# abstractguy/xagents

Hardware: AMD Instinct MI355X
Metric: env-steps/sec/GPU (PPO 16-env) + update ms; 1/2/4/8 MI355X (higher is better)
Workload: dtype f32; 1 GPU; PPO CartPole-v1, 16 envs/GPU, MLP[64,64], n_steps=128, 4 epochs x 4 minibatches, synthetic obs replay (the metric's 16-env configuration); the replay records ignore the actions, so the rollout runs its policy forwards as one batched launch (the `dynamics` object times the sequential step loop of an action-dependent env); n_envs_per_gpu=16, n_steps=128, batch_per_gpu=2048, minibatch_per_gpu=512, ppo_epochs=4, parallelism=dp1, graph=True, train_steps_per_graph_replay=8, update=persistent, allreduce=none

## Files before the change

xagents_amd/csrc/ppo_update_impl.hpp:

```cpp
#pragma once
#include <math.h>
#include <stdlib.h>

#include "../../include/xagents_hip.h"
#include "ppo_tile.hpp"
#include "xa_adam.hpp"
#include "xa_common.hpp"

__device__ void xa_forms_not_unrolled()
    __attribute__((error("ppo_update_kernel: the step loop's forms were not unrolled")));

namespace {

using namespace xa_ac;
using namespace xa_pt;

typedef __attribute__((address_space(1))) unsigned gu32;
typedef __attribute__((address_space(1))) unsigned long long gu64;

constexpr int kMaxSteps = 128;
constexpr int kCtlBytes = 256;
constexpr uint64_t kSpinTicks = 1000000000;
constexpr int kXcds = 8;
enum { kCntStats = 0, kAbort = 1 };
// ... 111 lines not shown
  return __longlong_as_double((long long)((u & ~1ull) | (unsigned long long)(tag & 1u)));
}
XA_DEV void st_d2_tagged(__amdgpu_buffer_rsrc_t r, uint32_t off, double a, double b, unsigned tag) {
  st_wt_d2(r, off, d_tagged(a, tag), d_tagged(b, tag));
}
XA_DEV bool d2_ok(const double2& v, unsigned tag) {
  return ((((unsigned)__double_as_longlong(v.x)) ^ tag) & 1u) == 0u &&
         ((((unsigned)__double_as_longlong(v.y)) ^ tag) & 1u) == 0u;
}

#ifndef XA_POLL_SLEEP
#define XA_POLL_SLEEP 1
#endif
template <int N>
XA_DEV bool poll_gran(__amdgpu_buffer_rsrc_t r, const uint32_t (&off)[N], int n, unsigned tag,
                      f32x4v (&v)[N], unsigned* ctl, unsigned epoch, int* status) {
  uint64_t t0 = 0;
  for (unsigned it = 0;; ++it) {
    const bool slow = (it & 15u) == 15u;
#pragma unroll
    for (int u = 0; u < N; ++u)
      if (u < n) v[u] = __builtin_amdgcn_raw_buffer_load_b128(r, off[u], 0, kAuxSc1);
    const unsigned ab = slow ? __hip_atomic_load((gu32*)(ctl + kAbort), __ATOMIC_RELAXED,
                                                 __HIP_MEMORY_SCOPE_AGENT)
                             : 0u;
    bool ok = true;
#pragma unroll
    for (int u = 0; u < N; ++u)
      if (u < n) ok = ok && gran_ok(v[u], tag);
    if (ok) return true;
    if (!slow) {
#ifndef XA_POLL_NOSLEEP
      __builtin_amdgcn_s_sleep(XA_POLL_SLEEP);
#endif
      continue;
    }
    if (ab == epoch) return false;
    {
      const uint64_t now = wall_clock64();
      if (t0 == 0) t0 = now;
      else if (now - t0 > kSpinTicks) {
        __hip_atomic_store((gu32*)(ctl + kAbort), epoch, __ATOMIC_RELAXED, __HIP_MEMORY_SCOPE_AGENT);
        if (status) __hip_atomic_store((gu32*)status, 1u, __ATOMIC_RELAXED, __HIP_MEMORY_SCOPE_AGENT);
        return false;
      }
    }
  }
}

template <int N>
XA_DEV bool poll_row(__amdgpu_buffer_rsrc_t r, const uint32_t (&off)[N], int n, unsigned tag,
                     RowG (&v)[N], unsigned* ctl, unsigned epoch, int* status) {
  uint64_t t0 = 0;
  for (unsigned it = 0;; ++it) {
    const bool slow = (it & 15u) == 15u;
#pragma unroll
    for (int u = 0; u < N; ++u)
      if (u < n) v[u] = ld_row(r, off[u]);
    const unsigned ab = slow ? __hip_atomic_load((gu32*)(ctl + kAbort), __ATOMIC_RELAXED,
                                                 __HIP_MEMORY_SCOPE_AGENT)
                             : 0u;
    bool ok = true;
#pragma unroll
    for (int u = 0; u < N; ++u)
      if (u < n) ok = ok && row_ok(v[u], tag);
    if (ok) return true;
    if (!slow) {
#ifndef XA_POLL_NOSLEEP
      __builtin_amdgcn_s_sleep(XA_POLL_SLEEP);
#endif
      continue;
    }
    if (ab == epoch) return false;
    {
      const uint64_t now = wall_clock64();
      if (t0 == 0) t0 = now;
      else if (now - t0 > kSpinTicks) {
        __hip_atomic_store((gu32*)(ctl + kAbort), epoch, __ATOMIC_RELAXED, __HIP_MEMORY_SCOPE_AGENT);
        if (status) __hip_atomic_store((gu32*)status, 1u, __ATOMIC_RELAXED, __HIP_MEMORY_SCOPE_AGENT);
        return false;
      }
    }
  }
}

template <int N>
XA_DEV bool poll_d2(__amdgpu_buffer_rsrc_t r, const uint32_t (&off)[N], uint32_t valid,
                    unsigned tag, double2 (&v)[N], unsigned* ctl, unsigned epoch, int* status) {
  uint64_t t0 = 0;
  for (unsigned it = 0;; ++it) {
    const bool slow = (it & 15u) == 15u;
#pragma unroll
    for (int u = 0; u < N; ++u)
      if ((valid >> u) & 1u) v[u] = ld_wt_d2(r, off[u]);
    const unsigned ab = slow ? __hip_atomic_load((gu32*)(ctl + kAbort), __ATOMIC_RELAXED,
                                                 __HIP_MEMORY_SCOPE_AGENT)
                             : 0u;
    bool ok = true;
#pragma unroll
    for (int u = 0; u < N; ++u)
      if ((valid >> u) & 1u) ok = ok && d2_ok(v[u], tag);
    if (ok) return true;
    if (!slow) {
#ifndef XA_POLL_NOSLEEP
      __builtin_amdgcn_s_sleep(XA_POLL_SLEEP);
#endif
      continue;
    }
    if (ab == epoch) return false;
    {
      const uint64_t now = wall_clock64();
      if (t0 == 0) t0 = now;
      else if (now - t0 > kSpinTicks) {
        __hip_atomic_store((gu32*)(ctl + kAbort), epoch, __ATOMIC_RELAXED, __HIP_MEMORY_SCOPE_AGENT);
        if (status) __hip_atomic_store((gu32*)status, 1u, __ATOMIC_RELAXED, __HIP_MEMORY_SCOPE_AGENT);
        return false;
      }
    }
  }
}

XA_DEV int xcc_id() {
  unsigned x;
  asm volatile("s_getreg_b32 %0, hwreg(HW_REG_XCC_ID)" : "=s"(x));
  return (int)(x & (kXcds - 1));
}

#ifdef XA_TRACE
constexpr int kTraceSteps = 32, kTracePts = 16;
__device__ unsigned xa_ppo_trace[256 * kTraceSteps * kTracePts];
#define XA_TRACE_PT(blk, k, i)                                                        \
  do {                                                                                \
    if (threadIdx.x == 0 && (k) < kTraceSteps) {                                      \
      unsigned long long t_;                                                          \
      asm volatile("s_memrealtime %0\n\ts_waitcnt lgkmcnt(0)" : "=s"(t_)::"memory");  \
      U.trace[(k) * kTracePts + (i)] = (unsigned)t_;                                  \
    }                                                                                 \
  } while (0)
#define XA_TRACE_CLK(blk, i)                                                          \
  do {                                                                                \
    if (threadIdx.x == 0) {                                                           \
      unsigned long long t_, c_;                                                      \
      asm volatile("s_memrealtime %0\n\ts_memtime %1\n\ts_waitcnt lgkmcnt(0)"        \
                   : "=s"(t_), "=s"(c_)::"memory");                                   \
      U.trace[(kTraceSteps - 1) * kTracePts + 8 + 2 * (i)] = (unsigned)t_;            \
      U.trace[(kTraceSteps - 1) * kTracePts + 9 + 2 * (i)] = (unsigned)c_;            \
    }                                                                                 \
  } while (0)
#define XA_TRACE_FLUSH(blk)                                                           \
  do {                                                                                \
    __syncthreads();                                                                  \
    for (int i_ = threadIdx.x; i_ < kTraceSteps * kTracePts; i_ += 256)              \
      xa_ppo_trace[(size_t)(blk) * kTraceSteps * kTracePts + i_] = U.trace[i_];      \
  } while (0)
#else
#define XA_TRACE_PT(blk, k, i) \
  do {                         \
  } while (0)
#define XA_TRACE_CLK(blk, i) \
  do {                       \
  } while (0)
#define XA_TRACE_FLUSH(blk) \
  do {                      \
  } while (0)
#endif

// ... 75 lines not shown
                    uint32_t (&w)[N], unsigned* ctl, unsigned epoch, int* status) {
  uint64_t t0 = 0;
  for (unsigned it = 0;; ++it) {
    const bool slow = (it & 15u) == 15u;
    bool ok = true;
#pragma unroll
    for (int u = 0; u < N; ++u)
      if (u < n) {
        const unsigned long long v = dp_ld(base, off[u]);
        w[u] = (uint32_t)v;
        ok = ok && (unsigned)(v >> 32) == tag;
      }
    const unsigned ab = slow ? __hip_atomic_load((gu32*)(ctl + kAbort), __ATOMIC_RELAXED,
                                                 __HIP_MEMORY_SCOPE_AGENT)
                             : 0u;
    if (ok) return true;
    if (slow) {
      if (ab == epoch) return false;
      const uint64_t now = wall_clock64();
      if (t0 == 0) t0 = now;
      else if (now - t0 > kSpinTicks) {
        __hip_atomic_store((gu32*)(ctl + kAbort), epoch, __ATOMIC_RELAXED, __HIP_MEMORY_SCOPE_AGENT);
        if (status) __hip_atomic_store((gu32*)status, 1u, __ATOMIC_RELAXED, __HIP_MEMORY_SCOPE_AGENT);
        return false;
      }
    }
    __builtin_amdgcn_s_sleep(XA_POLL_SLEEP);
  }
}

struct ShufKeys {
  uint32_t k[4];
  uint32_t half_bits;
};

XA_DEV ShufKeys shuf_keys(const XaShuffle& sh, uint64_t ctr, int epoch, int batch) {
  ShufKeys s;
  const xa_u4 r = xa_philox((uint32_t)epoch, 0x5u, (uint32_t)ctr, (uint32_t)(ctr >> 32),
                            (uint32_t)sh.seed, (uint32_t)(sh.seed >> 32));
  s.k[0] = r.x;
  s.k[1] = r.y;
  s.k[2] = r.z;
  s.k[3] = r.w;
  const uint32_t bits = batch <= 1 ? 1u : 32u - __clz((uint32_t)(batch - 1));
  s.half_bits = (bits + 1u) / 2u;
  if (s.half_bits == 0) s.half_bits = 1;
  return s;
}

XA_DEV int shuf_index(const XaShuffle& sh, const ShufKeys& keys, int epoch, int batch, int g) {
  if (sh.perm) return sh.perm[(size_t)epoch * batch + g];
  return (int)xa_permute((uint32_t)g, (uint32_t)batch, keys.half_bits, keys.k[0], keys.k[1],
                         keys.k[2], keys.k[3]);
}

constexpr int kPreBytes = 16384;
template <int OBS>
constexpr int pre_max() { return kPreBytes / ((OBS + 4) * 4); }

constexpr int kBF = 11;
template <int OBS, int A, int TS>
struct UpdLds {
  PtLds<OBS, A, TS> t;
  alignas(16) float row[(offs(OBS, A).P + 3) & ~3];
  alignas(16) float pre[pre_max<OBS>() * (OBS + 4)];
  alignas(16) float stage[TS * (OBS + 4)];
  alignas(16) float scr_own[TS == 32 ? 4 : 2 * 256 * kBF];
  XA_DEV float* scr() {
    static_assert(TS != 32 || (H + 2 * TS) * LDW + H * PtLds<OBS, A, TS>::LDT >= 2 * 256 * kBF,
                  "gather scratch");
    return TS == 32 ? t.sH1 : scr_own;
  }
  static constexpr int NS = 16 + Dims<OBS, A>::RPT, NQ4 = (NS + 3) / 4;
  float4 mv4[2][NQ4][256];
  float alpha[kMaxSteps];
  float stat[kMaxSteps][4];
  double red[256 * 4];
  double wsum[4];
  int flag;
  int xn[kXcds];
  int wx[4][kXcds];
  int xmem[256];
  int xrank;
#ifdef XA_TRACE
  unsigned trace[kTraceSteps * kTracePts];
#endif
};

constexpr int kLocForceWt = 2;

struct UniF {
  float b1, b2, eps, clip, omb1, omb2;
};
struct NoUniF {
  static constexpr float b1 = 0.0f, b2 = 0.0f, eps = 0.0f, clip = 0.0f, omb1 = 0.0f, omb2 = 0.0f;
};
XA_DEV float uni_vreg(float x) {
  float r;
  asm volatile("v_mov_b32 %0, %1" : "=v"(r) : "s"(x));
  return r;
}
XA_DEV float uni_clip_scale(float clip, float gn) {
  asm volatile("" : "+v"(clip));
  return clip > 0.0f ? clip * fminf(frcp(gn), frcp(clip)) : 1.0f;
}
template <bool ON>
XA_DEV int uni_tid(int tid) {
  if constexpr (ON) asm volatile("" : "+v"(tid));
  return tid;
}
template <bool ON>
XA_DEV auto uni_ptid(int tid) {
  if constexpr (ON) {
    asm volatile("" : "+v"(tid));
    return tid;
  } else {
    return PtOwnTid{};
  }
}


template <int BF>
struct FixShape {
  static constexpr int B = BF == 3 ? 2048 : 32768, MB = BF == 3 ? 512 : 8192, K = 16, NMB = 4;
  static constexpr int G = BF == 3 ? 32 : 256;
};
template <int OBS, int A, int TS, bool DP, bool PRE, int BF = 0>
__global__ __launch_bounds__(256) void ppo_update_kernel(XaPpoUpdateArgs p, Ws ws, int K_,
                                                          int n_mb_, int loc_) {
  constexpr bool FIX = BF == 3 || BF == 4;
  typedef FixShape<BF> FS;
  const int K = FIX ? FS::K : K_, n_mb = FIX ? FS::NMB : n_mb_;
  const int loc = (BF == 2 || BF == 4) ? 0 : loc_;
  if (loc && ((int)blockIdx.x & (kXcds - 1)) != 0) return;
  constexpr int RPT = Dims<OBS, A>::RPT;
  __shared__ __attribute__((aligned(16))) UpdLds<OBS, A, TS> U;
  PtLds<OBS, A, TS>& L = U.t;
  const Offs o = offs(OBS, A);
  const int P = o.P;
  const int tid = threadIdx.x, lane = tid & 63, w = tid >> 6;
  XA_STAMP_DECL
#ifdef XA_TRACE
  unsigned long long t_entry_;
  asm volatile("s_memrealtime %0\n\ts_waitcnt lgkmcnt(0)" : "=s"(t_entry_)::"memory");
#endif

  const unsigned gen =
      __hip_atomic_load((gu32*)ws.persist, __ATOMIC_RELAXED, __HIP_MEMORY_SCOPE_AGENT);
  const unsigned epoch = gen + 1u;
  const int xcc = xcc_id();
  const int G = FIX ? FS::G : loc ? p.n_blocks : (int)gridDim.x;
  const int b = loc ? (int)blockIdx.x / kXcds : (int)blockIdx.x;
#ifdef XA_TRACE
  if (tid == 0) U.trace[(kTraceSteps - 1) * kTracePts + 5] = (unsigned)t_entry_;
#endif
  constexpr int kSW = 2;
  const unsigned* const st_src = static_cast<const unsigned*>(p.stats_src);
  unsigned* const st_dst =
      p.stats_words > 0 ? static_cast<unsigned*>(p.stats_dst[gen % XA_PPO_STATS_SLOTS]) : nullptr;
  unsigned st_w[kSW];
#pragma unroll
  for (int u = 0; u < kSW; ++u) {
    const int i = b * 256 + tid + u * G * 256;
    st_w[u] = i < p.stats_words ? st_src[i] : 0u;
  }
  XA_STAMP_BLOCK(b == 0)
  XA_STAMP(30);
  XA_TRACE_PT(b, kTraceSteps - 1, 6);
  XA_TRACE_CLK(b, 0);
  const int B = FIX ? FS::B : p.batch, MB = FIX ? FS::MB : p.mb_size;
  const uint64_t ctr = p.shuffle.rng_counter ? *p.shuffle.rng_counter : 0ull;
  constexpr int RPT_ = Dims<OBS, A>::RPT;
  PSlice<OBS, A, TS> ps;
  ps.init(tid);
  float wv[16], rv[RPT_], mw[16], mr[RPT_], vw[16], vr[RPT_];
  ps.load(p.theta, wv, rv);
  ps.load(p.adam_m, mw, mr);
  ps.load(p.adam_v, vw, vr);
  bool kWt = (BF == 2 || BF == 4) ? loc_ == 0 : true;

  const bool two_level = BF == 2 || BF == 4 || (BF == 0 && !loc && TS == S && G >= kTwoLevelMinG);
  constexpr bool kOneRsrc = BF == 1 || BF == 3;
  const WsOff wo = ws_off(G, P, K);
  const __amdgpu_buffer_rsrc_t ws_r = rsrc(ws.ctl, (uint32_t)wo.total);
  const uint32_t cen_o = kOneRsrc ? (uint32_t)wo.cen_g : 0u, adv_o = kOneRsrc ? (uint32_t)wo.adv : 0u;
  const uint32_t rows_o = kOneRsrc ? (uint32_t)wo.rows_g : 0u, g_o = kOneRsrc ? (uint32_t)wo.g_g : 0u;
  const __amdgpu_buffer_rsrc_t cen_r = kOneRsrc ? ws_r : rsrc(ws.cen_g, (uint32_t)(G * 16));
  if ((two_level || loc) && tid == 0)
    st_gran2(cen_r, cen_o + (uint32_t)(16 * b), __uint_as_float((unsigned)xcc),
             __uint_as_float((unsigned)xcc), epoch, true);

  const int n_tiles_max = (min(MB, B) + TS - 1) / TS;
  const int TPB = (n_tiles_max + G - 1) / G;
  constexpr bool pre = PRE;
  const int t0 = *p.adam_step;
  for (int k = tid; k < K; k += 256)
    U.alpha[k] = adam_alpha(p.adam.lr, p.adam.beta1, p.adam.beta2, t0 + k + 1);
  float* const advs = reinterpret_cast<float*>(U.red);
  const __amdgpu_buffer_rsrc_t adv_r =
      kOneRsrc ? ws_r : rsrc(ws.adv, (uint32_t)((size_t)K * G * 16));
  const int per_k = TPB * TS;
  if (pre) {
    for (int i = tid; i < K * per_k; i += 256) {
      const int k = i / per_k, j = i - k * per_k;
      const int e = k / n_mb, m = k - e * n_mb;
      const int start = m * MB, cnt = min(MB, B - start);
      const int n_tiles = (cnt + TS - 1) / TS;
      const int mine = n_tiles > b ? (n_tiles - b + G - 1) / G : 0;
      const int q = (b + (j / TS) * G) * TS + (j % TS);
      float* slot = &U.pre[(size_t)i * (OBS + 4)];
      if (!(j < mine * TS && q < cnt)) {
#pragma unroll
        for (int kk = 0; kk < OBS + 4; ++kk) slot[kk] = 0.0f;
        slot[OBS] = -1.0f;
        advs[i] = 0.0f;
        continue;
      }
      const ShufKeys keys = shuf_keys(p.shuffle, ctr, e, B);
      const int idx = shuf_index(p.shuffle, keys, e, B, start + q);
      const float ret = p.returns[idx], oldv = p.old_values[idx];
      advs[i] = ret - oldv;
#pragma unroll
      for (int kk = 0; kk < OBS; ++kk) slot[kk] = p.obs[(size_t)idx * OBS + kk];
      slot[OBS] = (float)p.actions[idx];
      slot[OBS + 1] = ret;
      slot[OBS + 2] = oldv;
      slot[OBS + 3] = p.old_logp[idx];
    }
    __syncthreads();
  }
  XA_TRACE_PT(b, kTraceSteps - 1, 0);
  const bool grp0 = pre && per_k <= 32;
  if (grp0) {
    const int RL = per_k <= 16 ? 16 : 32, KPW = 64 / RL;
    const int g = lane / RL, j = lane - g * RL;
    for (int k0 = w; k0 < K; k0 += 4 * KPW) {
      const int k = k0 + 4 * g;
      double s1 = 0.0, s2 = 0.0;
      if (k < K && j < per_k) {
        const double a = (double)advs[k * per_k + j];
        s1 += a;
        s2 += a * a;
      }
      s1 = s1 + xa_dpp_f64<0xB1>(s1);
      s2 = s2 + xa_dpp_f64<0xB1>(s2);
      s1 = s1 + xa_dpp_f64<0x4E>(s1);
      s2 = s2 + xa_dpp_f64<0x4E>(s2);
      s1 = s1 + xa_dpp_f64<0x141>(s1);
      s2 = s2 + xa_dpp_f64<0x141>(s2);
      s1 = s1 + xa_dpp_f64<0x140>(s1);
      s2 = s2 + xa_dpp_f64<0x140>(s2);
      if (RL == 32) {
        s1 = s1 + xa_dpp_f64<0x142, 0xA>(s1);
        s2 = s2 + xa_dpp_f64<0x142, 0xA>(s2);
      }
      if (k < K && j == RL - 1) st_d2_tagged(adv_r, adv_o + (uint32_t)((k * G + b) * 16), s1, s2, epoch);
    }
  }
#ifndef XA_ABL_P0
  for (int k = w; k < K && !grp0; k += 4) {
#else
  for (int k = w; k < 0; k += 4) {
#endif
    if (pre) {
      double s1 = 0.0, s2 = 0.0;
      for (int j = lane; j < per_k; j += 64) {
        const double a = (double)advs[k * per_k + j];
        s1 += a;
        s2 += a * a;
      }
      s1 = xa_wave_sum_f64(s1);
      s2 = xa_wave_sum_f64(s2);
      if (lane == 0) st_d2_tagged(adv_r, adv_o + (uint32_t)((k * G + b) * 16), s1, s2, epoch);
      continue;
    }
    const int e = k / n_mb, m = k - e * n_mb;
    const int start = m * MB, cnt = min(MB, B - start);
    const int n_tiles = (cnt + TS - 1) / TS;
    const ShufKeys keys = shuf_keys(p.shuffle, ctr, e, B);
    const int mine = n_tiles > b ? (n_tiles - b + G - 1) / G : 0;
// ... 208 lines not shown
      const int start = m * MB, cnt = min(MB, B - start);
      const int q = tile * TS + tid;
      if (q < cnt) {
        const ShufKeys keys = shuf_keys(p.shuffle, ctr, e, B);
        idx = shuf_index(p.shuffle, keys, e, B, start + q);
      }
    }
    n_valid = idx >= 0;
    const size_t ix = idx >= 0 ? (size_t)idx : 0;
#pragma unroll
    for (int kk = 0; kk < OBS; ++kk) nx[kk] = idx >= 0 ? p.obs[ix * OBS + kk] : 0.0f;
    n_act = idx >= 0 ? (float)p.actions[ix] : 0.0f;
    n_ret = idx >= 0 ? p.returns[ix] : 0.0f;
    n_oldv = idx >= 0 ? p.old_values[ix] : 0.0f;
    n_oldlp = idx >= 0 ? p.old_logp[ix] : 0.0f;
  };
  fetch_tile(0, b);

  LossCfg cfg;
  cfg.is_ppo = true;
  cfg.has_adv_in = false;
  cfg.clip_norm = p.clip_norm;
  cfg.value_coef = p.value_coef;
  cfg.entropy_coef = p.entropy_coef;
  cfg.adv_eps = p.adv_eps;
  const float omb1 = 1.0f - p.adam.beta1, omb2 = 1.0f - p.adam.beta2;
  const int PP = padded(P), NP2 = PP / 2;
  const int CB = (NP2 + G - 1) / G;
  const int c0 = min(NP2, b * CB), nc = min(NP2, c0 + CB) - c0;
  const __amdgpu_buffer_rsrc_t rows_r =
      kOneRsrc ? ws_r : rsrc(ws.rows_g, (uint32_t)((size_t)G * PP * 8));
  const __amdgpu_buffer_rsrc_t g_r = kOneRsrc ? ws_r : rsrc(ws.g_g, (uint32_t)(PP * 8 + G * 64));
  const __amdgpu_buffer_rsrc_t xp_r = rsrc(ws.xpart_g, (uint32_t)(kXcds * PP * 16));
  float* srow = U.row;
  for (int i = P + tid; i < PP; i += 256) srow[i] = 0.0f;
  auto tag_of = [&](int k) { return gen * (unsigned)K + (unsigned)k + 1u; };
  float* const scr = U.scr();
  auto gather_rows = [&](__amdgpu_buffer_rsrc_t r, int nrow, int ncol, auto base,
                         unsigned tg) -> bool {
    const int total = nrow * ncol;
    uint32_t off[kBF];
    RowG x[kBF];
    int n = 0;
#pragma unroll
    for (int u = 0; u < kBF; ++u) {
      const int f = tid + 256 * u;
      const int rr = f / ncol;
      off[u] = f < total ? base(rr) + kRowPB * (uint32_t)(f - rr * ncol) : 0u;
      n += f < total;
    }
    const bool bad = !poll_row<kBF>(r, off, n, tg, x, ws.ctl, epoch, p.status);
#pragma unroll
    for (int u = 0; u < kBF; ++u)
      if (u < n) {
        const int f = tid + 256 * u;
        scr[2 * f] = row_v0(x[u]);
        scr[2 * f + 1] = row_v1(x[u]);
      }
    return bad;
  };

#ifndef XA_UNI_PRED
#define XA_UNI_PRED 1
#endif
#ifndef XA_UNI_FLOATS
#define XA_UNI_FLOATS 1
#endif
#ifndef XA_UNI_BLOCK
#define XA_UNI_BLOCK 1
#endif
  constexpr bool kUni = BF == 3 && !DP && OBS == 4 && A == 2;
  constexpr bool kUniP = kUni && XA_UNI_PRED, kUniF = kUni && XA_UNI_FLOATS;
  if constexpr (kUni && XA_UNI_BLOCK) __builtin_assume(b >= 0 && b < FS::G);
  [[maybe_unused]] std::conditional_t<kUniF, UniF, NoUniF> uf;
  if constexpr (kUniF) {
    cfg.clip_norm = uni_vreg(cfg.clip_norm);
    cfg.value_coef = uni_vreg(cfg.value_coef);
    cfg.entropy_coef = uni_vreg(cfg.entropy_coef);
    cfg.adv_eps = uni_vreg(cfg.adv_eps);
    uf.b1 = uni_vreg(p.adam.beta1), uf.b2 = uni_vreg(p.adam.beta2), uf.eps = uni_vreg(p.adam.eps);
    uf.clip = uni_vreg(p.adam.clip_norm), uf.omb1 = uni_vreg(omb1), uf.omb2 = uni_vreg(omb2);
  }
#define XA_UF(held, arg) (kUniF ? (held) : (arg))
  PtAcc<OBS, A> acc;
  float w2r[16];
  int k_tr = 0;
  auto stampf = [&](int slot) {
    XA_STAMP(slot);
    XA_TRACE_PT(b, k_tr, slot == 49 ? 15 : slot == 48 ? 7 : slot == 47 ? 6 : 8 + (slot - 50));
  };
  (void)k_tr;
  (void)stampf;
  constexpr int kForms = (BF == 1 || BF == 3) && !DP ? 3 : 1;
  const int form_sel =
      kForms == 1 || p.theta_trace || p.grad_trace || p.loss_out || p.grad_out ? 0 : kWt ? 1 : 2;
#define XA_OUT(f) ((kForms == 1 || form == 0) ? p.f : nullptr)
#pragma unroll kForms
  for (int form = 0; form < kForms; ++form) {
    if (kForms > 1 && !__builtin_constant_p(form)) xa_forms_not_unrolled();
    if (form != form_sel) continue;
    if (kForms > 1 && form != 0) kWt = form == 1;
    for (int k = 0; k < K; ++k) {
      if constexpr (kUniP) {
#pragma unroll
        for (int q = 0; q < RPT; ++q) asm volatile("" : "+v"(ps.rx[q]), "+v"(ps.rdst[q]));
      }
      const int m = k % n_mb;
      const int cnt = min(MB, B - m * MB);
      const int n_tiles = (cnt + TS - 1) / TS;
      const unsigned tag = tag_of(k);
      if constexpr (!kRegH1<OBS, A>) __syncthreads();
      cfg.adv_mean = U.stat[k][0];
      cfg.adv_std = U.stat[k][1];
      cfg.adv_rstd = U.stat[k][2];
      cfg.loss_scale = U.stat[k][3];
      acc.zero();
      if constexpr (!kRegH1<OBS, A>) load_w2_rows(L, w2r);
      if (XA_OUT(theta_trace) && b == 0) ps.store(XA_OUT(theta_trace) + (size_t)k * P, wv, rv);
      XA_STAMP(34);
      XA_TRACE_PT(b, k, 0);
      k_tr = k;
      const bool row_wt = kWt && !two_level;
      auto w2_out = [&](const PtAcc<OBS, A>& a) {
#ifndef XA_ABL_ROW
        pt_write_row_w2<OBS, A>(a, [&](int pr, float v0, float v1) {
          st_row(rows_r, rows_o + (uint32_t)((size_t)b * NP2 + pr) * kRowPB, v0, v1, tag, row_wt);
        });
#endif
      };
      for (int tile = b; tile < n_tiles; tile += G) {
        const bool last = tile + G >= n_tiles;
        if (pre) {
          XA_STAMP(35);
          const float* in = &U.pre[((size_t)k * TPB * TS + ((tile - b) / G) * TS) * (OBS + 4)];
#ifndef XA_ABL_TILE
          pt_tile<OBS, A, TS>(L, acc, cfg, in, wv, w2r, rv[0], rv[1], stampf, last, w2_out,
                              uni_ptid<kUniP>(tid));
#else
          if (last) w2_out(acc);
#endif
          XA_STAMP(36);
          XA_TRACE_PT(b, k, 14);
          continue;
        }
        __syncthreads();
        if (tid < TS) {
          float* rec = &U.stage[tid * (OBS + 4)];
#pragma unroll
          for (int kk = 0; kk < OBS; ++kk) rec[kk] = nx[kk];
          rec[OBS] = n_valid ? n_act : -1.0f;
          rec[OBS + 1] = n_ret;
          rec[OBS + 2] = n_oldv;
          rec[OBS + 3] = n_oldlp;
        }
        if (tile + G < n_tiles) fetch_tile(k, tile + G);
        __syncthreads();
        XA_STAMP(35);
        pt_tile<OBS, A, TS>(L, acc, cfg, U.stage, wv, w2r, rv[0], rv[1], stampf, last, w2_out);
        XA_STAMP(36);
      }
      if (b >= n_tiles) w2_out(acc);
      constexpr bool kRowDirect = TS == S;
#ifndef XA_ABL_ROW
      if constexpr (kRowDirect) {
        pt_write_row_rest<OBS, A>(acc, [&](int x, float v) {
          st_row1(rows_r, rows_o + (uint32_t)(((size_t)b * NP2 * 2 + x) * 4), v, tag, row_wt);
// ... 35 lines not shown
        if (flat && xnc > 0) {
          const bool bad = gather_rows(rows_r, ng, xnc, [&](int j) {
            return rows_o + (uint32_t)((size_t)U.xmem[j] * NP2 + xc0) * kRowPB;
          }, tag);
          if (__syncthreads_or(bad)) return;
          for (int c = tid; c < xnc; c += 256) {
            double t0 = 0.0, t1 = 0.0;
            for (int j = 0; j < ng; ++j) {
              t0 += (double)scr[2 * (j * xnc + c)];
              t1 += (double)scr[2 * (j * xnc + c) + 1];
            }
            st_d2_tagged(xp_r, (uint32_t)(((size_t)xcc * NP2 + xc0 + c) * 16), t0, t1, tag);
          }
          __syncthreads();
        }
        const int ncol = max(1, min(xnc, 256)), RG = 256 / ncol;
        const int rg = tid / ncol, cq = tid - rg * ncol;
        for (int cb = 0; !flat && cb < xnc; cb += ncol) {
          bool bad = false;
          if (rg < RG && cb + cq < xnc) {
            const int c = xc0 + cb + cq;
            double a0 = 0.0, a1 = 0.0;
            constexpr int kB = kBF;
            for (int j0 = rg; j0 < ng && !bad; j0 += RG * kB) {
              uint32_t off[kB];
              RowG x[kB];
              int n = 0;
#pragma unroll
              for (int u = 0; u < kB; ++u) {
                const int j = j0 + u * RG;
                off[u] = j < ng ? rows_o + (uint32_t)((size_t)U.xmem[j] * NP2 + c) * kRowPB : 0u;
                n += j < ng;
              }
              bad = !poll_row<kB>(rows_r, off, n, tag, x, ws.ctl, epoch, p.status);
#pragma unroll
              for (int u = 0; u < kB; ++u)
                if (u < n) {
                  a0 += (double)row_v0(x[u]);
                  a1 += (double)row_v1(x[u]);
                }
            }
            U.red[(rg * ncol + cq) * 2] = a0;
            U.red[(rg * ncol + cq) * 2 + 1] = a1;
          }
          if (__syncthreads_or(bad)) return;
          if (tid < ncol && cb + tid < xnc) {
            double t0 = 0.0, t1 = 0.0;
            for (int r = 0; r < RG; ++r) {
              t0 += U.red[(r * ncol + tid) * 2];
              t1 += U.red[(r * ncol + tid) * 2 + 1];
            }
            st_d2_tagged(xp_r, (uint32_t)(((size_t)xcc * NP2 + xc0 + cb + tid) * 16), t0, t1, tag);
          }
          __syncthreads();
        }
      }
      XA_STAMP(38);

      double sq = 0.0;
      auto publish = [&](int c, float g0, float g1) {
        const int cc = c0 + c;
        st_row(g_r, g_o + (uint32_t)cc * kRowPB, g0, g1, tag, kWt);
        if (XA_OUT(grad_out) && k == K - 1) {
          if (2 * cc < P) XA_OUT(grad_out)[canon_of_exchange<OBS, A>(2 * cc)] = g0;
          if (2 * cc + 1 < P) XA_OUT(grad_out)[canon_of_exchange<OBS, A>(2 * cc + 1)] = g1;
        }
        if (XA_OUT(grad_trace)) {
          float* gt = XA_OUT(grad_trace) + (size_t)k * P;
          if (2 * cc < P) gt[canon_of_exchange<OBS, A>(2 * cc)] = g0;
          if (2 * cc + 1 < P) gt[canon_of_exchange<OBS, A>(2 * cc + 1)] = g1;
        }
        sq += (double)g0 * (double)g0 + (double)g1 * (double)g1;
      };
      auto emit = [&](int c, float g0, float g1) {
        if constexpr (DP) {
          srow[2 * c] = g0;
          srow[2 * c + 1] = g1;
        } else {
          publish(c, g0, g1);
        }
      };
      const int parts_b = nc <= 128 ? min(4, 256 / max(nc, 1)) : 1;
      const bool col_b = !two_level && nc > 0 && parts_b > 1 && (G + parts_b - 1) / parts_b <= kBF;
      if (col_b) {
        double t0 = 0.0, t1 = 0.0;
        bool bad = false;
        if (uni_tid<kUniP>(tid) < parts_b * nc) {
          const int part = tid / nc, c = tid - part * nc;
          uint32_t off[kBF];
          RowG x[kBF];
          int n = 0;
#pragma unroll
          for (int u = 0; u < kBF; ++u) {
            const int r = part + parts_b * u;
            off[u] = r < G ? rows_o + (uint32_t)((size_t)r * NP2 + c0 + c) * kRowPB : 0u;
            n += r < G;
          }
          bad = !poll_row<kBF>(rows_r, off, n, tag, x, ws.ctl, epoch, p.status);
#pragma unroll
          for (int u = 0; u < kBF; ++u)
            if (u < n) {
              t0 += (double)row_v0(x[u]);
              t1 += (double)row_v1(x[u]);
            }
          U.red[(part * nc + c) * 2] = t0;
          U.red[(part * nc + c) * 2 + 1] = t1;
        }
        if (__syncthreads_or(bad)) return;
        for (int c = uni_tid<kUniP>(tid); c < nc; c += 256) {
          double s0 = 0.0, s1 = 0.0;
          for (int part = 0; part < parts_b; ++part) {
            s0 += U.red[(part * nc + c) * 2];
            s1 += U.red[(part * nc + c) * 2 + 1];
          }
          const float g0 = (float)s0, g1 = (float)s1;
          emit(c, g0, g1);
        }
      }
      constexpr bool flat_ok = BF == 0, gen_ok = BF != 1 && BF != 3;
      const bool flat_b = flat_ok && !col_b && !two_level && G * nc <= 256 * kBF;
      if (nc > 0 && flat_b) {
        const bool bad = gather_rows(rows_r, G, nc, [&](int r) {
          return rows_o + (uint32_t)((size_t)r * NP2 + c0) * kRowPB;
        }, tag);
        if (__syncthreads_or(bad)) return;
        const int parts = nc <= 128 ? min(4, 256 / nc) : 1;
#ifdef XA_ABL_BSUM
        if (false) {
#else
        if (parts > 1) {
#endif
          if (tid < parts * nc) {
            const int part = tid / nc, c = tid - part * nc;
            double t0 = 0.0, t1 = 0.0;
            for (int r = part; r < G; r += parts) {
              t0 += (double)scr[2 * (r * nc + c)];
              t1 += (double)scr[2 * (r * nc + c) + 1];
            }
            U.red[(part * nc + c) * 2] = t0;
            U.red[(part * nc + c) * 2 + 1] = t1;
          }
          __syncthreads();
        }
        for (int c = tid; c < nc; c += 256) {
          double t0 = 0.0, t1 = 0.0;
#ifdef XA_ABL_BSUM
          if (true) {
            t0 = scr[2 * c]; t1 = scr[2 * c + 1];
          } else
#endif
          if (parts > 1) {
            for (int part = 0; part < parts; ++part) {
              t0 += U.red[(part * nc + c) * 2];
              t1 += U.red[(part * nc + c) * 2 + 1];
            }
          } else {
            for (int r = 0; r < G; ++r) {
              t0 += (double)scr[2 * (r * nc + c)];
              t1 += (double)scr[2 * (r * nc + c) + 1];
            }
          }
          const float g0 = (float)t0, g1 = (float)t1;
          emit(c, g0, g1);
        }
      }
      if (gen_ok && nc > 0 && !flat_b && !col_b) {
        const int SRC = two_level ? kXcds : G;
        const int ncol = min(nc, 256), RG = min(SRC, 256 / ncol);
        const int rg = tid / ncol, cq = tid - rg * ncol;
        for (int cb = 0; cb < nc; cb += ncol) {
          bool bad = false;
          if (rg < RG && cb + cq < nc) {
            const int c = c0 + cb + cq;
            double a0 = 0.0, a1 = 0.0;
            constexpr int kB = 8;
            for (int j0 = rg; j0 < SRC && !bad; j0 += RG * kB) {
              uint32_t off[kB];
              int n = 0;
              if (two_level) {
                double2 x[kB];
#pragma unroll
                for (int u = 0; u < kB; ++u) off[u] = 0u;
                for (int u = 0; u < kB; ++u) {
                  const int xx = j0 + u * RG;
                  if (xx < kXcds && U.xn[xx] > 0) off[n++] = (uint32_t)(((size_t)xx * NP2 + c) * 16);
                }
                bad = !poll_d2<kB>(xp_r, off, (1u << n) - 1u, tag, x, ws.ctl, epoch, p.status);
                for (int u = 0; u < n; ++u) {
                  a0 += x[u].x;
                  a1 += x[u].y;
                }
// ... 11 lines not shown
                  if (u < n) {
                    a0 += (double)row_v0(xr[u]);
                    a1 += (double)row_v1(xr[u]);
                  }
              }
            }
            U.red[(rg * ncol + cq) * 2] = a0;
            U.red[(rg * ncol + cq) * 2 + 1] = a1;
          }
          if (__syncthreads_or(bad)) return;
          if (tid < ncol && cb + tid < nc) {
            double t0 = 0.0, t1 = 0.0;
            for (int r = 0; r < RG; ++r) {
              t0 += U.red[(r * ncol + tid) * 2];
              t1 += U.red[(r * ncol + tid) * 2 + 1];
            }
            const float g0 = (float)t0, g1 = (float)t1;
            emit(cb + tid, g0, g1);
          }
          __syncthreads();
        }
      }
      if constexpr (DP) {
        __syncthreads();
        const int par = k & 1;
        for (int c = tid; c < nc; c += 256) {
          const size_t o = dl.gsl + ((((size_t)par * G + b) * W + p.dp_rank) * CB0 + c) * 16;
          const uint32_t w0 = __float_as_uint(srow[2 * c]), w1 = __float_as_uint(srow[2 * c + 1]);
          for (int q = 0; q < W; ++q) {
            dp_st(p.dp_blocks[q], o, w0, tag);
            dp_st(p.dp_blocks[q], o + 8, w1, tag);
          }
        }
        bool bad = false;
        for (int c = tid; c < nc; c += 256) {
          constexpr int kW2 = 2 * XA_PPO_DP_MAX;
          size_t off[kW2];
          uint32_t x[kW2];
#pragma unroll
          for (int u = 0; u < kW2; ++u) {
            const int r = u >> 1;
            off[u] = r < W ? dl.gsl + ((((size_t)par * G + b) * W + r) * CB0 + c) * 16 + 8 * (u & 1)
                           : 0;
          }
          bad = bad || !dp_poll<kW2>(p.dp_blocks[p.dp_rank], off, 2 * W, tag, x, ws.ctl, epoch,
                                     p.status);
          double s0 = 0.0, s1 = 0.0;
          for (int r = 0; r < W; ++r) {
            s0 += (double)__uint_as_float(x[2 * r]);
            s1 += (double)__uint_as_float(x[2 * r + 1]);
          }
          publish(c, (float)s0, (float)s1);
        }
        if (__syncthreads_or(bad)) return;
      }
      (void)sq;
      XA_STAMP(40);
      XA_TRACE_PT(b, k, 3);

      float gw[16], gr[RPT];
      double tot = 0.0;
      bool bad = false;
      float bm[4 * NQ4], bv[4 * NQ4];
#pragma unroll
      for (int q4 = 0; q4 < NQ4; ++q4) {
        const float4 a = U.mv4[0][q4][tid], c = U.mv4[1][q4][tid];
        const xa_f2 b1 = {XA_UF(uf.b1, p.adam.beta1), XA_UF(uf.b1, p.adam.beta1)};
        const xa_f2 b2 = {XA_UF(uf.b2, p.adam.beta2), XA_UF(uf.b2, p.adam.beta2)};
        const xa_f2 m01 = xa_f2{a.x, a.y} * b1, m23 = xa_f2{a.z, a.w} * b1;
        const xa_f2 v01 = xa_f2{c.x, c.y} * b2, v23 = xa_f2{c.z, c.w} * b2;
        bm[4 * q4] = m01.x; bm[4 * q4 + 1] = m01.y; bm[4 * q4 + 2] = m23.x; bm[4 * q4 + 3] = m23.y;
        bv[4 * q4] = v01.x; bv[4 * q4 + 1] = v01.y; bv[4 * q4 + 2] = v23.x; bv[4 * q4 + 3] = v23.y;
      }
      {
        constexpr int NG = 8 + RPT;
        uint32_t off[NG];
        RowG x[NG];
#pragma unroll
        for (int h = 0; h < 8; ++h) off[h] = g_o + (uint32_t)((256 * h + tid) * kRowPB);
#pragma unroll
        for (int q = 0; q < RPT; ++q)
          off[8 + q] = g_o + (uint32_t)((ps.rx[q] >= 0 ? ps.rx[q] / 2 : 0) * kRowPB);
        bad = !poll_row<NG>(g_r, off, NG, tag, x, ws.ctl, epoch, p.status);
        XA_STAMP(46);
#pragma unroll
        for (int h = 0; h < 8; ++h) {
          gw[2 * h] = row_v0(x[h]);
          gw[2 * h + 1] = row_v1(x[h]);
        }
#pragma unroll
        for (int q = 0; q < RPT; ++q)
          gr[q] = ps.rx[q] >= 0 ? ((ps.rx[q] & 1) ? row_v1(x[8 + q]) : row_v0(x[8 + q])) : 0.0f;
      }
      {
        double s0 = 0.0, s1 = 0.0;
#pragma unroll
        for (int q = 0; q < 16; q += 2) {
          s0 = fma((double)gw[q], (double)gw[q], s0);
          s1 = fma((double)gw[q + 1], (double)gw[q + 1], s1);
        }
#pragma unroll
        for (int q = 0; q < RPT; ++q) s0 = fma((double)gr[q], (double)gr[q], s0);
        const double ws = xa_wave_sum_f64(s0 + s1);
        if ((uni_tid<kUniP>(tid) & 63) == 0) U.wsum[w] = ws;
      }
      if (__syncthreads_or(bad)) return;
      XA_STAMP(47);
      XA_TRACE_PT(b, k, 4);
#ifndef XA_ABL_CNORM
      tot = (U.wsum[0] + U.wsum[1]) + (U.wsum[2] + U.wsum[3]);
      const float gn = __builtin_amdgcn_sqrtf((float)tot);
      const float sc = XA_UF(uni_clip_scale(uf.clip, gn),
                             p.adam.clip_norm > 0.0f
                                 ? p.adam.clip_norm * fminf(frcp(gn), frcp(p.adam.clip_norm)) : 1.0f);
#else
      const float sc = (float)tot;
#endif
      const float alpha = U.alpha[k];
#ifndef XA_ABL_ADAM
      {
        const xa_f2 k1 = {sc * XA_UF(uf.omb1, omb1), sc * XA_UF(uf.omb1, omb1)};
        const xa_f2 k2 = {(sc * sc) * XA_UF(uf.omb2, omb2), (sc * sc) * XA_UF(uf.omb2, omb2)};
        const xa_f2 al = {alpha, alpha}, ep = {XA_UF(uf.eps, p.adam.eps), XA_UF(uf.eps, p.adam.eps)};
        float th[4 * NQ4];
#pragma unroll
        for (int q = 0; q < 4 * NQ4; ++q) th[q] = q < 16 ? wv[q] : q < NS ? rv[q - 16] : 0.0f;
#pragma unroll
        for (int q = 0; q < NS; q += 2) {
          const xa_f2 g = {q < 16 ? gw[q] : gr[q - 16], q + 1 < 16 ? gw[q + 1] : q + 1 < NS ? gr[q + 1 - 16] : 0.0f};
          const xa_f2 mn = xa_fma2(g, k1, xa_f2{bm[q], bm[q + 1]});
          const xa_f2 vn = xa_fma2(g * g, k2, xa_f2{bv[q], bv[q + 1]});
          const xa_f2 step = mn * al;
          const xa_f2 den = xa_f2{__builtin_amdgcn_sqrtf(vn.x), __builtin_amdgcn_sqrtf(vn.y)} + ep;
          const xa_f2 r = {__builtin_amdgcn_rcpf(den.x), __builtin_amdgcn_rcpf(den.y)};
          const xa_f2 tn = xa_fma2(-step, r, xa_f2{th[q], th[q + 1]});
          th[q] = tn.x;
          th[q + 1] = tn.y;
          bm[q] = mn.x;
          bm[q + 1] = mn.y;
          bv[q] = vn.x;
          bv[q + 1] = vn.y;
        }
#pragma unroll
        for (int q = 0; q < 16; ++q) wv[q] = th[q];
#pragma unroll
        for (int q = 0; q < RPT; ++q) rv[q] = th[16 + q];
#pragma unroll
        for (int q4 = 0; q4 < NQ4; ++q4) {
          U.mv4[0][q4][tid] = make_float4(bm[4 * q4], bm[4 * q4 + 1], bm[4 * q4 + 2], bm[4 * q4 + 3]);
          U.mv4[1][q4][tid] = make_float4(bv[4 * q4], bv[4 * q4 + 1], bv[4 * q4 + 2], bv[4 * q4 + 3]);
        }
      }
#endif
#ifndef XA_ABL_LDS
      ps.to_lds(L, wv, rv);
#endif
      XA_STAMP(43);
      XA_TRACE_PT(b, k, 5);
    }
  }
#undef XA_OUT
#undef XA_UF
  XA_TRACE_CLK(b, 1);
  XA_TRACE_FLUSH(b);
  if (tid % G == b % 256) {
    ps.store(p.theta, wv, rv);
    float mw[16], mr[RPT], vw[16], vr[RPT];
#pragma unroll
    for (int q = 0; q < NS; ++q) {
      const float4 a = U.mv4[0][q >> 2][tid], c = U.mv4[1][q >> 2][tid];
      const float mq = (q & 3) == 0 ? a.x : (q & 3) == 1 ? a.y : (q & 3) == 2 ? a.z : a.w;
      const float vq = (q & 3) == 0 ? c.x : (q & 3) == 1 ? c.y : (q & 3) == 2 ? c.z : c.w;
      if (q < 16) {
        mw[q] = mq;
        vw[q] = vq;
      } else {
        mr[q - 16] = mq;
        vr[q - 16] = vq;
      }
    }
    ps.store(p.adam_m, mw, mr);
    ps.store(p.adam_v, vw, vr);
  }
  if (b == 0) {
    if (tid == 0) {
      *p.adam_step = t0 + K;
      if (p.bump_counter && p.shuffle.rng_counter)
        *const_cast<uint64_t*>(p.shuffle.rng_counter) = ctr + 1;
      __hip_atomic_store((gu32*)ws.persist, epoch, __ATOMIC_RELAXED, __HIP_MEMORY_SCOPE_AGENT);
    }
  }
}

template <int OBS, int A>
int occupancy_min() {
  void* const kernels[] = {
      (void*)ppo_update_kernel<OBS, A, S, false, false>, (void*)ppo_update_kernel<OBS, A, 16, false, false>,
      (void*)ppo_update_kernel<OBS, A, S, true, false>, (void*)ppo_update_kernel<OBS, A, 16, true, false>,
      (void*)ppo_update_kernel<OBS, A, S, false, true>, (void*)ppo_update_kernel<OBS, A, 16, false, true>,
      (void*)ppo_update_kernel<OBS, A, S, true, true>, (void*)ppo_update_kernel<OBS, A, 16, true, true>,
      (void*)ppo_update_kernel<OBS, A, 16, false, false, 1>,
      (void*)ppo_update_kernel<OBS, A, 16, true, false, 1>,
      (void*)ppo_update_kernel<OBS, A, 16, false, true, 1>,
      (void*)ppo_update_kernel<OBS, A, 16, true, true, 1>,
      (void*)ppo_update_kernel<OBS, A, 16, false, true, 3>,
      (void*)ppo_update_kernel<OBS, A, S, false, true, 4>,
      (void*)ppo_update_kernel<OBS, A, 16, true, true, 3>,
      (void*)ppo_update_kernel<OBS, A, S, true, true, 4>,
      (void*)ppo_update_kernel<OBS, A, S, false, false, 2>,
      (void*)ppo_update_kernel<OBS, A, S, true, false, 2>,
      (void*)ppo_update_kernel<OBS, A, S, false, true, 2>,
      (void*)ppo_update_kernel<OBS, A, S, true, true, 2>};
  int occ = 1 << 30;
  for (void* k : kernels) {
    int o = 0;
    if (hipOccupancyMaxActiveBlocksPerMultiprocessor(&o, k, 256, 0) != hipSuccess) return 0;
    occ = min(occ, o);
  }
  return occ;
}

template <int OBS, int A>
int capacity() {
  static int cap[64] = {0};
  int dev = 0;
  if (hipGetDevice(&dev) != hipSuccess || dev < 0 || dev >= 64) return 0;
  if (cap[dev] == 0) {
    int cus = 0;
    if (hipDeviceGetAttribute(&cus, hipDeviceAttributeMultiprocessorCount, dev) != hipSuccess)
      return 0;
    cap[dev] = cus * occupancy_min<OBS, A>();
  }
  return cap[dev];
}


int tile_samples(int mb_size, int G) { return G > (mb_size + S - 1) / S ? 16 : S; }

bool use_local(const XaPpoUpdateArgs* a, int G, int cap) {
  static const int env = [] {
    const char* e = getenv("XA_PPO_LOCAL");
    return e && e[0] == '0' ? 0 : 1;
  }();
  if (!env || a->placement == XA_PPO_PLACE_SPREAD) return false;
  if (a->dp_world > 1 && a->placement != XA_PPO_PLACE_LOCAL &&
      a->placement != XA_PPO_PLACE_LOCAL_WT)
    return false;
  return G < kTwoLevelMinG && G < 64 && (long)G * kXcds <= (long)cap;
}

bool col_b_everywhere(int G, int P) {
  const int NP2 = padded(P) / 2, CB = (NP2 + G - 1) / G;
  for (int b = 0; b < G; ++b) {
    const int c0 = min(NP2, b * CB), nc = min(NP2, c0 + CB) - c0;
    if (nc <= 0) continue;
    const int parts = nc <= 128 ? min(4, 256 / nc) : 1;
    if (!(parts > 1 && (G + parts - 1) / parts <= kBF)) return false;
  }
  return true;
}

template <int OBS, int A, int TS>
void launch_ts(const XaPpoUpdateArgs* a, int G, bool dp, bool loc, const Ws& ws, int K, int n_mb,
               hipStream_t s) {
  const dim3 grid(loc ? G * kXcds : G);
  const int n_tiles_max = (min(a->mb_size, a->batch) + TS - 1) / TS;
  const int TPB = (n_tiles_max + G - 1) / G;
  const bool pre = K * TPB * TS <= pre_max<OBS>();
  const int l = !loc ? 0 : a->placement == XA_PPO_PLACE_LOCAL_WT ? kLocForceWt : 1;
  static const bool fix_on = [] {
    const char* e = getenv("XA_PPO_FIXED_SHAPE");
    return !(e && e[0] == '0');
  }();
  auto is_fix = [&](auto fs) {
    typedef decltype(fs) F;
    return fix_on && pre && G == F::G && K == F::K && n_mb == F::NMB && a->batch == F::B &&
           a->mb_size == F::MB;
  };
  if constexpr (TS == 16) {
    if (col_b_everywhere(G, offs(OBS, A).P)) {
      if (is_fix(FixShape<3>{}) && dp)
        hipLaunchKernelGGL((ppo_update_kernel<OBS, A, TS, true, true, 3>), grid, dim3(256), 0, s, *a, ws, K, n_mb, l);
      else if (is_fix(FixShape<3>{}))
        hipLaunchKernelGGL((ppo_update_kernel<OBS, A, TS, false, true, 3>), grid, dim3(256), 0, s, *a, ws, K, n_mb, l);
      else if (dp && pre)
        hipLaunchKernelGGL((ppo_update_kernel<OBS, A, TS, true, true, 1>), grid, dim3(256), 0, s, *a, ws, K, n_mb, l);
      else if (dp)
        hipLaunchKernelGGL((ppo_update_kernel<OBS, A, TS, true, false, 1>), grid, dim3(256), 0, s, *a, ws, K, n_mb, l);
      else if (pre)
        hipLaunchKernelGGL((ppo_update_kernel<OBS, A, TS, false, true, 1>), grid, dim3(256), 0, s, *a, ws, K, n_mb, l);
      else
        hipLaunchKernelGGL((ppo_update_kernel<OBS, A, TS, false, false, 1>), grid, dim3(256), 0, s, *a, ws, K, n_mb, l);
      return;
    }
  } else {
    if (!loc && G >= kTwoLevelMinG) {
      if (is_fix(FixShape<4>{}) && dp)
        hipLaunchKernelGGL((ppo_update_kernel<OBS, A, TS, true, true, 4>), grid, dim3(256), 0, s, *a, ws, K, n_mb, l);
      else if (is_fix(FixShape<4>{}))
        hipLaunchKernelGGL((ppo_update_kernel<OBS, A, TS, false, true, 4>), grid, dim3(256), 0, s, *a, ws, K, n_mb, l);
      else if (dp && pre)
        hipLaunchKernelGGL((ppo_update_kernel<OBS, A, TS, true, true, 2>), grid, dim3(256), 0, s, *a, ws, K, n_mb, l);
      else if (dp)
        hipLaunchKernelGGL((ppo_update_kernel<OBS, A, TS, true, false, 2>), grid, dim3(256), 0, s, *a, ws, K, n_mb, l);
      else if (pre)
        hipLaunchKernelGGL((ppo_update_kernel<OBS, A, TS, false, true, 2>), grid, dim3(256), 0, s, *a, ws, K, n_mb, l);
      else
        hipLaunchKernelGGL((ppo_update_kernel<OBS, A, TS, false, false, 2>), grid, dim3(256), 0, s, *a, ws, K, n_mb, l);
      return;
    }
  }
  if (dp && pre)
    hipLaunchKernelGGL((ppo_update_kernel<OBS, A, TS, true, true>), grid, dim3(256), 0, s, *a, ws, K, n_mb, l);
  else if (dp)
    hipLaunchKernelGGL((ppo_update_kernel<OBS, A, TS, true, false>), grid, dim3(256), 0, s, *a, ws, K, n_mb, l);
  else if (pre)
    hipLaunchKernelGGL((ppo_update_kernel<OBS, A, TS, false, true>), grid, dim3(256), 0, s, *a, ws, K, n_mb, l);
  else
    hipLaunchKernelGGL((ppo_update_kernel<OBS, A, TS, false, false>), grid, dim3(256), 0, s, *a, ws, K, n_mb, l);
}

template <int OBS, int A>
int launch(const XaPpoUpdateArgs* a, int G, int K, int n_mb, hipStream_t s) {
  const int P = offs(OBS, A).P;
  const Ws ws = carve(a->workspace, G, P, K);
  const bool loc = use_local(a, G, capacity<OBS, A>());
  if (tile_samples(a->mb_size, G) == 16)
    launch_ts<OBS, A, 16>(a, G, a->dp_world > 1, loc, ws, K, n_mb, s);
  else
    launch_ts<OBS, A, S>(a, G, a->dp_world > 1, loc, ws, K, n_mb, s);
  XA_CHECK_LAUNCH("xa_ppo_update");
  return 0;
}

}

#define XA_PPO_SHAPE_TU(O, A_)                                                               \
  int xa_ppo_capacity_##O##_##A_() { return capacity<O, A_>(); }                            \
  int xa_ppo_launch_##O##_##A_(const XaPpoUpdateArgs* a, int G, int K, int n_mb,            \
                               hipStream_t s) {                                             \
// ... 7 lines not shown
```

Before: 15.47 million env-steps/s.

## Reduce column partials within a wave and replace block barriers with sticky abort vote

For the column-form update kernels, each wave now polls its own column rows and reduces the per-part partial sums with cross-lane permutes. This replaces writing partials to LDS followed by a block-wide barrier and a second reduction pass. Failure votes use a sticky LDS abort flag read with readfirstlane instead of __syncthreads_or, and polling re-issues loads only for rows that are not ready yet. The trade-offs are more permute traffic and a narrower eligibility check on column counts per wave. Abort detection is deferred to the later barrier, which could delay error exits.

```diff
diff --git a/xagents_amd/csrc/ppo_update_impl.hpp b/xagents_amd/csrc/ppo_update_impl.hpp
--- a/xagents_amd/csrc/ppo_update_impl.hpp
+++ b/xagents_amd/csrc/ppo_update_impl.hpp
@@ -217,6 +217,69 @@
       }
     }
   }
+}
+
+XA_DEV double lane_f64(double v, int src) {
+  const unsigned long long u = (unsigned long long)__double_as_longlong(v);
+  const unsigned lo = (unsigned)__builtin_amdgcn_ds_bpermute(src << 2, (int)(unsigned)u);
+  const unsigned hi = (unsigned)__builtin_amdgcn_ds_bpermute(src << 2, (int)(unsigned)(u >> 32));
+  return __longlong_as_double((long long)(((unsigned long long)hi << 32) | lo));
+}
+
+template <int N>
+XA_DEV bool poll_row_missing(__amdgpu_buffer_rsrc_t r, const uint32_t (&off)[N], int n,
+                             unsigned tag, RowG (&v)[N], unsigned* ctl, unsigned epoch,
+                             int* status) {
+  {
+#pragma unroll
+    for (int u = 0; u < N; ++u)
+      if (u < n) v[u] = ld_row(r, off[u]);
+    bool ok = true;
+#pragma unroll
+    for (int u = 0; u < N; ++u)
+      if (u < n) ok = ok && row_ok(v[u], tag);
+    if (ok) return true;
+#ifndef XA_POLL_NOSLEEP
+    __builtin_amdgcn_s_sleep(XA_POLL_SLEEP);
+#endif
+  }
+  uint64_t t0 = 0;
+  for (unsigned it = 1;; ++it) {
+    const bool slow = (it & 15u) == 15u;
+#pragma unroll
+    for (int u = 0; u < N; ++u)
+      if (u < n && !row_ok(v[u], tag)) v[u] = ld_row(r, off[u]);
+    const unsigned ab = slow ? __hip_atomic_load((gu32*)(ctl + kAbort), __ATOMIC_RELAXED,
+                                                 __HIP_MEMORY_SCOPE_AGENT)
+                             : 0u;
+    bool ok = true;
+#pragma unroll
+    for (int u = 0; u < N; ++u)
+      if (u < n) ok = ok && row_ok(v[u], tag);
+    if (ok) return true;
+    if (!slow) {
+#ifndef XA_POLL_NOSLEEP
+      __builtin_amdgcn_s_sleep(XA_POLL_SLEEP);
+#endif
+      continue;
+    }
+    if (ab == epoch) return false;
+    {
+      const uint64_t now = wall_clock64();
+      if (t0 == 0) t0 = now;
+      else if (now - t0 > kSpinTicks) {
+        __hip_atomic_store((gu32*)(ctl + kAbort), epoch, __ATOMIC_RELAXED, __HIP_MEMORY_SCOPE_AGENT);
+        if (status) __hip_atomic_store((gu32*)status, 1u, __ATOMIC_RELAXED, __HIP_MEMORY_SCOPE_AGENT);
+        return false;
+      }
+    }
+  }
+}
+template <bool MISSING, int N>
+XA_DEV bool poll_row_col(__amdgpu_buffer_rsrc_t r, const uint32_t (&off)[N], int n, unsigned tag,
+                         RowG (&v)[N], unsigned* ctl, unsigned epoch, int* status) {
+  if constexpr (MISSING) return poll_row_missing<N>(r, off, n, tag, v, ctl, epoch, status);
+  else return poll_row<N>(r, off, n, tag, v, ctl, epoch, status);
 }
 
 template <int N>
@@ -458,6 +521,7 @@
   int wx[4][kXcds];
   int xmem[256];
   int xrank;
+  int abort;
 #ifdef XA_TRACE
   unsigned trace[kTraceSteps * kTracePts];
 #endif
@@ -495,6 +559,21 @@
   }
 }
 
+template <class LDS>
+XA_DEV int sticky_vote(LDS& U, bool bad) {
+  if (bad) U.abort = 1;
+  __syncthreads();
+  return __builtin_amdgcn_readfirstlane(U.abort);
+}
+#ifndef XA_PHB_ABORT
+#define XA_PHB_ABORT 1
+#endif
+#ifndef XA_PHB_WAVE
+#define XA_PHB_WAVE 1
+#endif
+#ifndef XA_PHB_REPOLL
+#define XA_PHB_REPOLL 1
+#endif
 
 template <int BF>
 struct FixShape {
@@ -506,6 +585,10 @@
                                                           int n_mb_, int loc_) {
   constexpr bool FIX = BF == 3 || BF == 4;
   typedef FixShape<BF> FS;
+  constexpr bool kPhb = (BF == 1 || BF == 3) && !DP;
+  constexpr bool kPhbAbort = kPhb && XA_PHB_ABORT, kPhbWave = kPhb && XA_PHB_WAVE;
+  constexpr bool kPhbRepoll = kPhb && XA_PHB_REPOLL;
+  static_assert(!kPhb || TS == 16, "the column-form kernels run 16-sample tiles");
   const int K = FIX ? FS::K : K_, n_mb = FIX ? FS::NMB : n_mb_;
   const int loc = (BF == 2 || BF == 4) ? 0 : loc_;
   if (loc && ((int)blockIdx.x & (kXcds - 1)) != 0) return;
@@ -572,6 +655,9 @@
   const int t0 = *p.adam_step;
   for (int k = tid; k < K; k += 256)
     U.alpha[k] = adam_alpha(p.adam.lr, p.adam.beta1, p.adam.beta2, t0 + k + 1);
+  if constexpr (kPhbAbort) {
+    if (tid == 0) U.abort = 0;
+  }
   float* const advs = reinterpret_cast<float*>(U.red);
   const __amdgpu_buffer_rsrc_t adv_r =
       kOneRsrc ? ws_r : rsrc(ws.adv, (uint32_t)((size_t)K * G * 16));
@@ -946,6 +1032,7 @@
     uf.clip = uni_vreg(p.adam.clip_norm), uf.omb1 = uni_vreg(omb1), uf.omb2 = uni_vreg(omb2);
   }
 #define XA_UF(held, arg) (kUniF ? (held) : (arg))
+#define XA_VOTE(bad) (kPhbAbort ? sticky_vote(U, bad) : __syncthreads_or(bad))
   PtAcc<OBS, A> acc;
   float w2r[16];
   int k_tr = 0;
@@ -1147,7 +1234,49 @@
       };
       const int parts_b = nc <= 128 ? min(4, 256 / max(nc, 1)) : 1;
       const bool col_b = !two_level && nc > 0 && parts_b > 1 && (G + parts_b - 1) / parts_b <= kBF;
-      if (col_b) {
+      [[maybe_unused]] bool bad_b = false;
+      if constexpr (kPhbWave) {
+        const int t = uni_tid<kUniP>(tid), bl = t & 63;
+        const int bw = __builtin_amdgcn_readfirstlane(t >> 6);
+        const int cpw = parts_b == 2 ? 32 : parts_b == 3 ? 21 : 16;
+        if (nc > 0 && bw * cpw < nc) {
+          const int part = (bl >= cpw) + (bl >= 2 * cpw) + (bl >= 3 * cpw);
+          const int j = bl - part * cpw, c = bw * cpw + j;
+          double t0 = 0.0, t1 = 0.0;
+          if (part < parts_b && c < nc) {
+            uint32_t off[kBF];
+            RowG x[kBF];
+            int n = 0;
+#pragma unroll
+            for (int u = 0; u < kBF; ++u) {
+              const int r = part + parts_b * u;
+              off[u] = r < G ? rows_o + (uint32_t)((size_t)r * NP2 + c0 + c) * kRowPB : 0u;
+              n += r < G;
+            }
+            bad_b = !poll_row_col<kPhbRepoll, kBF>(rows_r, off, n, tag, x, ws.ctl, epoch, p.status);
+#pragma unroll
+            for (int u = 0; u < kBF; ++u)
+              if (u < n) {
+                t0 += (double)row_v0(x[u]);
+                t1 += (double)row_v1(x[u]);
+              }
+          }
+          const bool wave_bad = __ballot(bad_b) != 0ull;
+          double s0 = 0.0, s1 = 0.0;
+          s0 += t0;
+          s1 += t1;
+#pragma unroll
+          for (int q = 1; q < 4; ++q)
+            if (q < parts_b) {
+              s0 += lane_f64(t0, j + q * cpw);
+              s1 += lane_f64(t1, j + q * cpw);
+            }
+          if (!wave_bad && bl < cpw && c < nc) {
+            const float g0 = (float)s0, g1 = (float)s1;
+            emit(c, g0, g1);
+          }
+        }
+      } else if (col_b) {
         double t0 = 0.0, t1 = 0.0;
         bool bad = false;
         if (uni_tid<kUniP>(tid) < parts_b * nc) {
@@ -1161,7 +1290,7 @@
             off[u] = r < G ? rows_o + (uint32_t)((size_t)r * NP2 + c0 + c) * kRowPB : 0u;
             n += r < G;
           }
-          bad = !poll_row<kBF>(rows_r, off, n, tag, x, ws.ctl, epoch, p.status);
+          bad = !poll_row_col<kPhbRepoll, kBF>(rows_r, off, n, tag, x, ws.ctl, epoch, p.status);
 #pragma unroll
           for (int u = 0; u < kBF; ++u)
             if (u < n) {
@@ -1171,7 +1300,7 @@
           U.red[(part * nc + c) * 2] = t0;
           U.red[(part * nc + c) * 2 + 1] = t1;
         }
-        if (__syncthreads_or(bad)) return;
+        if (XA_VOTE(bad)) return;
         for (int c = uni_tid<kUniP>(tid); c < nc; c += 256) {
           double s0 = 0.0, s1 = 0.0;
           for (int part = 0; part < parts_b; ++part) {
@@ -1349,6 +1478,7 @@
         for (int q = 0; q < RPT; ++q)
           off[8 + q] = g_o + (uint32_t)((ps.rx[q] >= 0 ? ps.rx[q] / 2 : 0) * kRowPB);
         bad = !poll_row<NG>(g_r, off, NG, tag, x, ws.ctl, epoch, p.status);
+        if constexpr (kPhbWave) bad = bad || bad_b;
         XA_STAMP(46);
 #pragma unroll
         for (int h = 0; h < 8; ++h) {
@@ -1371,7 +1501,7 @@
         const double ws = xa_wave_sum_f64(s0 + s1);
         if ((uni_tid<kUniP>(tid) & 63) == 0) U.wsum[w] = ws;
       }
-      if (__syncthreads_or(bad)) return;
+      if (XA_VOTE(bad)) return;
       XA_STAMP(47);
       XA_TRACE_PT(b, k, 4);
 #ifndef XA_ABL_CNORM
@@ -1428,6 +1558,7 @@
   }
 #undef XA_OUT
 #undef XA_UF
+#undef XA_VOTE
   XA_TRACE_CLK(b, 1);
   XA_TRACE_FLUSH(b);
   if (tid % G == b % 256) {
@@ -1523,6 +1654,7 @@
     if (nc <= 0) continue;
     const int parts = nc <= 128 ? min(4, 256 / nc) : 1;
     if (!(parts > 1 && (G + parts - 1) / parts <= kBF)) return false;
+    if (nc > 4 * (64 / parts)) return false;
   }
   return true;
 }
```

New measurement: 17.32 million env-steps/s, median of 6. +12.0%, better.
